# KwonGihyun/TweedieMix

Hardware: AMD Instinct MI355X
Metric: denoise steps/sec @ SDXL 1024^2 K=3 concepts (fusion phase); images/sec at 1/2/4/8 GPUs (higher is better)
Workload: dtype bf16

## Files before the change

### tweediemix_amd/csrc/gemm_kernel.h

```cpp
#pragma once
#include "common.h"
#include <type_traits>
#include <stdlib.h>
#include <atomic>

namespace tmix_gemm {

constexpr int BK = 64;

static __device__ __forceinline__ float xor32_sum(float x) {
    auto r = __builtin_amdgcn_permlane32_swap(__float_as_uint(x), __float_as_uint(x), false, false);
    return __uint_as_float(r[0]) + __uint_as_float(r[1]);
}

template <int CTRL> static __device__ __forceinline__ float dpp_row(float x) {
    return __int_as_float(__builtin_amdgcn_update_dpp(0, __float_as_int(x), CTRL, 0xf, 0xf, false));
}
static __device__ __forceinline__ float swap32_sum(float a, float b) {
    auto r = __builtin_amdgcn_permlane32_swap(__float_as_uint(a), __float_as_uint(b), false, false);
    return __uint_as_float(r[0]) + __uint_as_float(r[1]);
}
static __device__ __forceinline__ float swap16_sum(float a, float b) {
    auto r = __builtin_amdgcn_permlane16_swap(__float_as_uint(a), __float_as_uint(b), false, false);
    return __uint_as_float(r[0]) + __uint_as_float(r[1]);
}

struct Params {
    const bf16_t* A; int64_t lda, strideA;
    const bf16_t* W; int64_t ldw, strideW;
    bf16_t* C; int64_t ldc, strideC;
    const float* bias; int64_t strideBias;
    const bf16_t* R; int64_t ldr, strideR;
    const float* rgb; int rows_per_group;
    bf16_t* Ct; int64_t ldct, strideCt; int n_trans_begin;
    int M, N, K, tiles_m, tiles_n, group_m, epilogue;
    unsigned bytesA, bytesW;
    float* stats_out; int64_t strideStatsOut, ldStatsOut;
    const float* ln_stats; int64_t strideLnStats, ldLnStats; const float* ln_colsum; int64_t strideLnColsum;
    float ln_inv_c, ln_eps; int ln_parts;
    int H, Wd, Cin, Ho, Wo, mode, ntaps;
    int up_hw; unsigned up_magic;
    unsigned long long* prof; int prof_detail;
    int wide;
    const unsigned char* scaleA; const unsigned char* scaleW; int64_t strideScaleA, strideScaleW;
    int64_t ldScaleA;
    unsigned char* scale_out; int64_t ldScaleOut; int f8out;
    unsigned char* f8copy; int64_t ldF8copy;
    const char* pf; long long pf_bytes;
    int pf_per;
    int w_period, w_groups; unsigned w_magic;
    float* cs_out;
    const bf16_t* S1; const bf16_t* S2; int c1s, c2s; unsigned bytesS1, bytesS2;
};

static __device__ __forceinline__ void blds16(__amdgpu_buffer_rsrc_t rsrc, unsigned voff, unsigned soff, char* lds_dst) {
    __builtin_amdgcn_raw_ptr_buffer_load_lds(rsrc, (__attribute__((address_space(3))) void*)lds_dst, 16, voff, soff, 0, 0);
}

constexpr int f8_block_cap(int bn) { return bn >= 256 ? 88 : 224; }

template <int N> static __device__ __forceinline__ void wait_vmcnt() { asm volatile("s_waitcnt vmcnt(%0)" ::"n"(N) : "memory"); }

constexpr int PFU = 8;
#define TMIX_PF_TOUCH(p, pf_keep, touches, nth_, idx)                                                                                                     \
    unsigned pf_keep[PFU];                                                                                                                                \
    _Pragma("unroll") for (int pf_u_ = 0; pf_u_ < PFU; ++pf_u_) pf_keep[pf_u_] = 0;                                                                       \
    if ((p).pf && (touches)) {                                                                                                                            \
        const long long pf_nwg_ = (long long)gridDim.x * gridDim.y, pf_nth_ = (nth_);                                                                     \
        const long long pf_lines_ = ((p).pf_bytes + 127) >> 7; const int pf_per_ = (p).pf_per;                                      \
        const long long pf_first_ = ((long long)blockIdx.y * gridDim.x + blockIdx.x) * pf_nth_ + (idx);                                                   \
        _Pragma("unroll") for (int pf_u_ = 0; pf_u_ < PFU; ++pf_u_) {                                                                                     \
            const long long pf_ln_ = pf_first_ + (long long)pf_u_ * pf_nwg_ * pf_nth_;                                                                    \
            if (pf_u_ < pf_per_ && pf_ln_ < pf_lines_)                                                                                                    \
                asm volatile("global_load_dword %0, %1, off" : "=v"(pf_keep[pf_u_]) : "v"((p).pf + (pf_ln_ << 7)) : "memory");                            \
        }                                                                                                                                                 \
    }
static __device__ __forceinline__ void pf_keep_alive(const unsigned (&pf_keep)[PFU]) {
#pragma unroll
    for (int u = 0; u < PFU; ++u) asm volatile("" :: "v"(pf_keep[u]));
}

struct TileId { int tile_m, tile_n, by; };
static __device__ __forceinline__ TileId tile_of_workgroup(const Params& p) {
    int bid, by;
    xcd_remap_grid(bid, by);
    const int per_group = p.group_m * p.tiles_n;
    const int grp = bid / per_group;
    const int first_m = grp * p.group_m;
    const int gsize = min(p.tiles_m - first_m, p.group_m);
    const int rem = bid - grp * per_group;
    const int tile_n = rem / gsize, tile_m = first_m + (rem - tile_n * gsize);
// ... 334 lines not shown
            }
        }
    };

    if constexpr (LW) {
        if (loader) {
            constexpr int PRE = NS >= 4 ? 2 : NS - 1;
#pragma unroll
            for (int s = 0; s < PRE; ++s)
                if (s < nk) stage(s, s);
            if (nk >= PRE) wait_vmcnt<(PRE - 1) * L>(); else wait_vmcnt<0>();
            pf_keep_alive(pf_keep);
            __builtin_amdgcn_s_barrier();
#pragma unroll
            for (int s = PRE; s < NS - 1; ++s)
                if (s < nk) stage(s, s);
            int nxt = NS - 1;
            for (int kt = 0; kt < nk; ++kt) {
                const bool more = kt + NS - 1 < nk;
                if (more) stage(nxt, kt + NS - 1);
                if (more) wait_vmcnt<(NS - 2) * L>(); else wait_vmcnt<0>();
                __builtin_amdgcn_s_barrier();
                nxt = (nxt + 1 == NS) ? 0 : nxt + 1;
            }
            if (p.stats_out) __syncthreads();
            return;
        }
    }

    uint4* ln_mfrag = (uint4*)(smem + RING);
    uint4* ln_cfrag = ln_mfrag + BM;
    float* ln_rs = (float*)(ln_cfrag + BN);
    float* bias_lds = ln_rs + BM;
    float bias_r = 0.f;
    if (p.bias && tid < BN && n0 + tid < p.N) bias_r = (p.bias + (int64_t)bzw * p.strideBias)[n0 + tid];
    float* rgb_lds = bias_lds + BN;
    float rgb_r = 0.f;
    bool rgb_one = true;
    if constexpr (CONV) {
        if (p.rgb) {
            const int g0 = m0 / p.rows_per_group;
            rgb_one = (min(m0 + BM, p.M) - 1) / p.rows_per_group == g0;
            if (rgb_one && tid < BN && n0 + tid < p.N) rgb_r = p.rgb[(int64_t)g0 * p.N + n0 + tid];
        }
    }
    constexpr int PU = 16;
    typedef __attribute__((ext_vector_type(2))) unsigned u32x2;
    u32x2 lnv[PU];
    float ln_cs = 0.f;
    const bool ln_on = p.ln_stats != nullptr;
    if (ln_on) {
        const __amdgpu_buffer_rsrc_t rsS = __builtin_amdgcn_make_buffer_rsrc((void*)(p.ln_stats + (int64_t)bz * p.strideLnStats), 0,
                                                                              (int)(p.ln_parts * p.ldLnStats * 8), 0x00020000);
        if (tid < BM) {
            const int lnm = min(m0 + tid, p.M - 1);
#pragma unroll
            for (int q = 0; q < PU; ++q)
                if (q < p.ln_parts) lnv[q] = __builtin_amdgcn_raw_buffer_load_b64(rsS, lnm * 8, q * (int)p.ldLnStats * 8, 0);
        }
        if (tid < BN) ln_cs = (p.ln_colsum + (int64_t)bzw * p.strideLnColsum)[min(n0 + tid, p.N - 1)];
    }
    auto ln_reduce = [&]() {
        if (tid < BN) { bias_lds[tid] = bias_r; if constexpr (CONV) rgb_lds[tid] = rgb_r; }
        if (!ln_on) return;
        if (tid < BM) {
            float s1 = 0.f, s2 = 0.f;
#pragma unroll
            for (int q = 0; q < PU; ++q)
                if (q < p.ln_parts) { s1 += __uint_as_float(lnv[q].x); s2 += __uint_as_float(lnv[q].y); }
            const float mean = s1 * p.ln_inv_c;
            ln_rs[tid] = rsqrtf(fmaxf(s2 * p.ln_inv_c - mean * mean, 0.f) + p.ln_eps);
            ln_mfrag[tid] = ln_mean_operand(-mean);
        }
        if (tid < BN) ln_cfrag[tid] = ln_colsum_operand(ln_cs);
    };

    f32x16 acc[FM][FN];
#pragma unroll
    for (int i = 0; i < FM; ++i)
#pragma unroll
        for (int j = 0; j < FN; ++j)
#pragma unroll
            for (int r = 0; r < 16; ++r) acc[i][j][r] = 0.f;

    const bool trans = (EK == 1 || EK == 2 || EK == 4) ? false : (p.n_trans_begin >= 0) && (n0 >= p.n_trans_begin);
    constexpr bool SQ = (FM == FN && TM == TN) && !PH;
    const bool tswap = trans && SQ;
    const int l31 = lane & 31, lhi = lane >> 5;
    const int fsw = (lane >> 1) & 7;

    const int offA = (wr * TM + l31) * 128, offW = A_TILE + (wc * TN + l31) * 128;
    const int off_a = tswap ? offW : offA, off_b = tswap ? offA : offW;
    const bf16_t* Rb = p.R ? p.R + (int64_t)bz * p.strideR : nullptr;
    const bool plain_epi = EK ? false : !trans && p.epilogue != TMIX_EPI_GEGLU && !(p.wide & 1);
    constexpr bool PREF = FM * FN <= 4;
    uint2 rres[PREF ? FM : 1][PREF ? FN : 1][4];
    auto prefetch_residual = [&]() {
        if constexpr (PREF)
#pragma unroll
        for (int i = 0; i < FM; ++i) {
            int m = m0 + wr * TM + i * 32 + l31; if (m > p.M - 1) m = p.M - 1;
#pragma unroll
            for (int j = 0; j < FN; ++j)
#pragma unroll
                for (int g = 0; g < 4; ++g) {
                    int n = n0 + wc * TN + j * 32 + g * 8 + lhi * 4; if (n > p.N - 4) n = p.N - 4;
                    rres[i][j][g] = *(const uint2*)(Rb + (int64_t)m * p.ldr + n);
                }
        }
    };
    constexpr int WP_I = (FN / 2) * 4 + (FN & 1) * 2;
    constexpr bool WPREF = FM * WP_I <= 12 && !(CONV && F8L && LW);
    uint4 rw[WPREF ? FM * WP_I : 1];
    const bool wide_res = EK != 1 && WPREF && Rb && (EK >= 2 || (p.wide & 1)) && kg == 0;
    auto prefetch_residual_wide = [&]() {
        if constexpr (WPREF) {
            auto grab = [&](int j0, int base, auto cf_tag) {
                constexpr int CF = decltype(cf_tag)::value, CW = CF * 32, LPR = CW / 8, RPI = 64 / LPR, NP = 32 / RPI;
                const int rr = lane / LPR, nc = n0 + wc * TN + j0 * 32 + (lane % LPR) * 8;
#pragma unroll
                for (int i = 0; i < FM; ++i)
#pragma unroll
                    for (int ps = 0; ps < NP; ++ps) {
                        const int m = m0 + wr * TM + i * 32 + ps * RPI + rr;
                        if (m < p.M && nc < p.N) rw[i * WP_I + base + ps] = *(const uint4*)(Rb + (int64_t)m * p.ldr + nc);
                    }
            };
#pragma unroll
            for (int c = 0; c < FN / 2; ++c) grab(c * 2, c * 4, std::integral_constant<int, 2>{});
            if constexpr (FN & 1) grab(FN - 1, (FN / 2) * 4, std::integral_constant<int, 1>{});
        }
    };
    auto epi_prefetch = [&]() __attribute__((always_inline)) {
        if constexpr (WPREF) {
            if (wide_res) prefetch_residual_wide();
            else {
#pragma unroll
                for (int q = 0; q < FM * WP_I; ++q) rw[q] = make_uint4(0u, 0u, 0u, 0u);
            }
        }
    };
    if constexpr (PHL) {
        constexpr int PL = PA + PB;
        static_assert(2 * PL <= 63, "vmcnt immediate");
        const int ns = p.K / (64 / EB);
        const int offA4 = (wr * TM + l31) * 64, offW4 = BM * 64 + (wc * TN + l31) * 64;
        typedef int v8i_t __attribute__((ext_vector_type(8)));
        int f8sA[F8 ? FM : 1], f8sW[F8 ? FN : 1];
        if constexpr (F8) {
            const unsigned char* sa = p.scaleA + (int64_t)bz * p.strideScaleA;
            const unsigned char* sw = p.scaleW + (int64_t)bzw * p.strideScaleW;
#pragma unroll
            for (int i = 0; i < FM; ++i) f8sA[i] = F8B ? 0 : (int)(sa[min(m0 + wr * TM + i * 32 + l31, p.M - 1)] * 0x01010101u);
#pragma unroll
            for (int j = 0; j < FN; ++j) f8sW[j] = (int)(sw[min(n0 + wc * TN + j * 32 + l31, p.N - 1)] * 0x01010101u);
        }
        char* const scl = smem + RING + (BM + BN) * 16 + BM * 4 + BN * 4;
        if constexpr (F8B) {
            const int nblk = p.K / 32;
            const __amdgpu_buffer_rsrc_t rsS = __builtin_amdgcn_make_buffer_rsrc((void*)p.scaleA, 0, (int)((int64_t)nblk * p.ldScaleA), 0x00020000);
            const unsigned lane_off = (unsigned)((lane * 16) / BM) * (unsigned)p.ldScaleA + (unsigned)((lane * 16) % BM)
                                    + (unsigned)(bz * p.strideScaleA + m0);
            const int npcs = (nblk * BM + 1023) / 1024;
            for (int q = w; q < npcs; q += NW)
                blds16(rsS, lane_off + (unsigned)(q * (1024 / BM)) * (unsigned)p.ldScaleA, 0u, scl + q * 1024);
        }
        const int f4 = (lane >> 2) & 3;
        const int q0 = ((0 + lhi) ^ f4) << 4, q1 = ((2 + lhi) ^ f4) << 4;
        const int grp = w >> 2;
#pragma unroll
        for (int s = 0; s < 3; ++s)
            if (s < ns) ph_stage(s, s);
        ln_reduce();
        if (ns >= 3) wait_vmcnt<2 * PL>(); else if (ns == 2) wait_vmcnt<PL>(); else wait_vmcnt<0>();
        __builtin_amdgcn_s_barrier();
        asm volatile("" ::: "memory");
        if (prof_on) pt1 = prof_now();
        pf_keep_alive(pf_keep);
        if (grp) { __builtin_amdgcn_s_barrier(); asm volatile("" ::: "memory"); }
        auto slice = [&](int s, auto stage_tag) {
            constexpr bool ST = decltype(stage_tag)::value;
            const char* pa = smem + (s & 3) * SLOT + offA4;
            const char* pw = smem + (s & 3) * SLOT + offW4;
            frag_ab a[2][FM], b[2][FN];
            v8i_t a8[F8 ? FM : 1], b8[F8 ? FN : 1];
            int f8use[F8B ? FM : 1];
            if constexpr (F8) {
                const int c0 = (lhi ^ f4) << 4, c1 = ((2 + lhi) ^ f4) << 4;
#pragma unroll
                for (int i = 0; i < FM; ++i) {
                    const uint4 lo = *(const uint4*)(pa + i * 32 * 64 + c0), hi = *(const uint4*)(pa + i * 32 * 64 + c1);
                    a8[i] = (v8i_t){(int)lo.x, (int)lo.y, (int)lo.z, (int)lo.w, (int)hi.x, (int)hi.y, (int)hi.z, (int)hi.w};
                }
#pragma unroll
                for (int j = 0; j < FN; ++j) {
                    const uint4 lo = *(const uint4*)(pw + j * 32 * 64 + c0), hi = *(const uint4*)(pw + j * 32 * 64 + c1);
                    b8[j] = (v8i_t){(int)lo.x, (int)lo.y, (int)lo.z, (int)lo.w, (int)hi.x, (int)hi.y, (int)hi.z, (int)hi.w};
                }
            } else {
#pragma unroll
            for (int i = 0; i < FM; ++i) { a[0][i] = *(const frag_ab*)(pa + i * 32 * 64 + q0); a[1][i] = *(const frag_ab*)(pa + i * 32 * 64 + q1); }
#pragma unroll
            for (int j = 0; j < FN; ++j) { b[0][j] = *(const frag_ab*)(pw + j * 32 * 64 + q0); b[1][j] = *(const frag_ab*)(pw + j * 32 * 64 + q1); }
            }
            if constexpr (F8B) {
#pragma unroll
                for (int i = 0; i < FM; ++i)
                    f8use[i] = (int)((unsigned)(unsigned char)scl[(2 * s + lhi) * BM + wr * TM + i * 32 + l31] * 0x01010101u);
            }
            if (s + 2 < ns) wait_vmcnt<PL>(); else wait_vmcnt<0>();
            if (PREF && s == ns - 1 && Rb && plain_epi) prefetch_residual();
            if (s == ns - 1) epi_prefetch();
            asm volatile("s_waitcnt lgkmcnt(0)" ::: "memory");
            __builtin_amdgcn_sched_barrier(0);
            __builtin_amdgcn_s_barrier();
            __builtin_amdgcn_sched_barrier(0);
            __builtin_amdgcn_s_setprio(1);
            char* sA = smem + ((s + 3) & 3) * SLOT;
            char* sW = sA + BM * 64;
            constexpr int KSTEPS = F8 ? 1 : 2;
            constexpr int NMF = KSTEPS * FM * FN, GAP = NMF / PL;
            int issued = 0;
#pragma unroll
            for (int kk = 0; kk < KSTEPS; ++kk)
#pragma unroll
                for (int i = 0; i < FM; ++i)
#pragma unroll
                    for (int j = 0; j < FN; ++j) {
                        if constexpr (F8) acc[i][j] = __builtin_amdgcn_mfma_scale_f32_32x32x64_f8f6f4(b8[j], a8[i], acc[i][j], 0, 0, 0, f8sW[j], 0, F8B ? f8use[i] : f8sA[i]);
                        else acc[i][j] = __builtin_amdgcn_mfma_f32_32x32x16_bf16(b[kk][j], a[kk][i], acc[i][j], 0, 0, 0);
                        const int idx = (kk * FM + i) * FN + j;
                        if constexpr (ST) {
                            if (idx % GAP == (GAP > 1 ? 1 : 0) && issued < PL) {
                                __builtin_amdgcn_sched_barrier(0);
                                if (issued < PA) blds16(rsA, phA[issued], (unsigned)(s + 3) * 64u, sA + (issued * NW + w) * 1024);
                                else             blds16(rsW, phW[issued - PA], (unsigned)(s + 3) * 64u, sW + ph_w(issued - PA) * 1024);
                                __builtin_amdgcn_sched_barrier(0);
                                ++issued;
                            }
                        }
                    }
            __builtin_amdgcn_s_setprio(0);
            __builtin_amdgcn_sched_barrier(0);
            __builtin_amdgcn_s_barrier();
            __builtin_amdgcn_sched_barrier(0);
            asm volatile("" ::: "memory");
        };
        int s = 0;
        for (; s + 3 < ns; ++s) slice(s, std::true_type{});
        for (; s < ns; ++s) slice(s, std::false_type{});
        if (!grp) { __builtin_amdgcn_s_barrier(); asm volatile("" ::: "memory"); }
    } else
    {
    if constexpr (!LW) {
#pragma unroll
        for (int s = 0; s < NS - 1; ++s)
            if (s < nk) stage(s, s);
    }
    ln_reduce();
    if constexpr (!LW) { if (nk >= NS - 1) wait_vmcnt<(NS - 2) * L>(); else wait_vmcnt<0>(); }
    __builtin_amdgcn_s_barrier();
    asm volatile("" ::: "memory");
    if (prof_on) pt1 = prof_now();
    pf_keep_alive(pf_keep);
    int cur = 0, nxt = NS - 1;
    constexpr int KPW = F8L ? 2 : 4 / KS;
    const int k0 = kg * KPW;
    typedef int v8i_t __attribute__((ext_vector_type(8)));
    typedef std::conditional_t<F8L, v8i_t, frag_ab> frag_t;
    frag_t fa[2][FM], fb[2][FN];
    int f8a[2][(F8L && F8B) ? FM : 1];
    int f8sA[(F8L && !F8B) ? FM : 1], f8sW[F8L ? FN : 1];
    if constexpr (F8L) {
        const unsigned char* swp_ = p.scaleW + (int64_t)bzw * p.strideScaleW;
#pragma unroll
        for (int j = 0; j < FN; ++j) f8sW[j] = (int)(swp_[min(n0 + wc * TN + j * 32 + l31, p.N - 1)] * 0x01010101u);
        if constexpr (!F8B) {
            const unsigned char* sap_ = p.scaleA + (int64_t)bz * p.strideScaleA;
#pragma unroll
            for (int i = 0; i < FM; ++i) f8sA[i] = (int)(sap_[min(m0 + wr * TM + i * 32 + l31, p.M - 1)] * 0x01010101u);
        }
    }
    auto rdfrag = [&](const char* row, int kk) __attribute__((always_inline)) -> frag_t {
        if constexpr (F8L) {
            const uint4 lo = *(const uint4*)(row + (((4 * kk + lhi) ^ fsw) << 4)), hi = *(const uint4*)(row + (((4 * kk + 2 + lhi) ^ fsw) << 4));
            return (v8i_t){(int)lo.x, (int)lo.y, (int)lo.z, (int)lo.w, (int)hi.x, (int)hi.y, (int)hi.z, (int)hi.w};
        } else {
            return *(const frag_ab*)(row + ((((k0 + kk) * 2 + lhi) ^ fsw) << 4));
        }
    };
    auto rdscale = [&](int rbuf, int kk, int i) __attribute__((always_inline)) -> int {
        if constexpr (CONV) return (int)((unsigned)(unsigned char)smem[rbuf * STAGE + A_TILE + B_TILE + (wr * TM + i * 32 + l31) * 4 + 2 * kk + lhi] * 0x01010101u);
        else return (int)((unsigned)(unsigned char)smem[rbuf * STAGE + A_TILE + B_TILE + (2 * kk + lhi) * BM + wr * TM + i * 32 + l31] * 0x01010101u);
    };
    auto mma = [&](f32x16& c, const frag_t& b_, const frag_t& a_, int j, int i, int S) __attribute__((always_inline)) {
        if constexpr (F8L) c = __builtin_amdgcn_mfma_scale_f32_32x32x64_f8f6f4(b_, a_, c, 0, 0, 0, f8sW[j], 0, F8B ? f8a[S][F8B ? i : 0] : f8sA[F8B ? 0 : i]);
        else c = __builtin_amdgcn_mfma_f32_32x32x16_bf16(b_, a_, c, 0, 0, 0);
    };
    constexpr int NMF = FM * FN, NRD = FM + FN;
    constexpr bool ROLL = (NW * KS > 4 && NMF * 16 + 2 * NRD * 4 > 200) || (F8L && LW);
    auto kstep = [&](const int S, const int rbuf, const int rkk, const int nd, const int dbuf, const int dkt) {
        const char* pa = smem + rbuf * STAGE + off_a;
        const char* pb = smem + rbuf * STAGE + off_b;
        char* sA = smem + dbuf * STAGE;
        constexpr int RPQ = (NRD + NMF - 1) / NMF;
        const int dpq = (nd + NMF - 1) / NMF;
#pragma unroll
        for (int q = 0; q < NMF; ++q) {
            const int i = ROLL ? q % FM : q / FN, j = ROLL ? q / FM : q - (q / FN) * FN;
            const int SB = ROLL ? 0 : S;
            mma(acc[i][j], fb[SB][j], fa[S][i], j, i, S);
            __builtin_amdgcn_sched_barrier(0);
            if constexpr (ROLL) {
                if (q < FM) { fa[1 - S][q] = rdfrag(pa + q * 32 * 128, rkk); if constexpr (F8L && F8B) f8a[1 - S][q] = rdscale(rbuf, rkk, q); }
                if (i == FM - 1) fb[0][j] = rdfrag(pb + j * 32 * 128, rkk);
            } else {
#pragma unroll
                for (int u = 0; u < RPQ; ++u) {
                    const int r = q * RPQ + u;
                    if (r < FM) { fa[1 - S][r] = rdfrag(pa + r * 32 * 128, rkk); if constexpr (F8L && F8B) f8a[1 - S][r] = rdscale(rbuf, rkk, r); }
                    else if (r < NRD) fb[1 - S][r - FM] = rdfrag(pb + (r - FM) * 32 * 128, rkk);
                }
            }
            if constexpr (!CONV && !LW) {
#pragma unroll
                for (int u = 0; u < dpq; ++u) {
                    const int r = q * dpq + u;
                    if (r < nd) dma_piece(r, sA, dkt);
                }
            }
            __builtin_amdgcn_sched_barrier(0);
        }
    };
    auto ktile = [&](int kt, auto more_tag) {
        constexpr bool MORE = decltype(more_tag)::value && !LW;
        if constexpr (CONV && MORE) { stage(nxt, kt + NS - 1); __builtin_amdgcn_sched_barrier(0); }
        if constexpr (!decltype(more_tag)::value) {
            if (PREF && kt == nk - 1 && Rb && plain_epi) prefetch_residual();
            if (kt == nk - 1) epi_prefetch();
            __builtin_amdgcn_sched_barrier(0);
        }
#pragma unroll
        for (int kk = 0; kk < KPW - 1; ++kk)
            kstep(kk & 1, cur, kk + 1, (kk == 0 && MORE && !CONV) ? L : 0, nxt, kt + NS - 1);
        if constexpr (KPW == 1 && !CONV && MORE) { stage(nxt, kt + NS - 1); __builtin_amdgcn_sched_barrier(0); }
        asm volatile("s_waitcnt lgkmcnt(0)" ::: "memory");
        if constexpr (!LW) { if constexpr (MORE) wait_vmcnt<(NS - 2) * L>(); else { if (kt + 1 < nk) wait_vmcnt<0>(); } }
        __builtin_amdgcn_sched_barrier(0);
        __builtin_amdgcn_s_barrier();
        __builtin_amdgcn_sched_barrier(0);
        asm volatile("" ::: "memory");
        cur = (cur + 1 == NS) ? 0 : cur + 1;
        nxt = (nxt + 1 == NS) ? 0 : nxt + 1;
        kstep((KPW - 1) & 1, cur, 0, 0, 0, 0);
    };
    static_assert(KPW == 1 || ((KPW - 1) & 1) == 1, "the next tile's first fragments go to register set 0");
#pragma unroll
    for (int r = 0; r < NRD; ++r) {
        if (r < FM) { fa[0][r] = rdfrag(smem + off_a + r * 32 * 128, 0); if constexpr (F8L && F8B) f8a[0][r] = rdscale(0, 0, r); }
        else fb[0][r - FM] = rdfrag(smem + off_b + (r - FM) * 32 * 128, 0);
    }
    int kt = 0;
    for (; kt + NS - 1 < nk; ++kt) ktile(kt, std::true_type{});
    for (; kt < nk; ++kt) ktile(kt, std::false_type{});
    }

    if constexpr (KS > 1) {
        float4* xch = (float4*)smem + (size_t)wm_ * (FM * FN * 4 * 64) + lane;
        if (kg == 1) {
#pragma unroll
            for (int i = 0; i < FM; ++i)
#pragma unroll
                for (int j = 0; j < FN; ++j)
#pragma unroll
                    for (int g = 0; g < 4; ++g)
                        xch[((i * FN + j) * 4 + g) * 64] = make_float4(acc[i][j][g * 4], acc[i][j][g * 4 + 1], acc[i][j][g * 4 + 2], acc[i][j][g * 4 + 3]);
        }
        __syncthreads();
        if (kg == 1) {
            __syncthreads();
            if (p.stats_out) __syncthreads();
            return;
        }
#pragma unroll
        for (int i = 0; i < FM; ++i)
#pragma unroll
            for (int j = 0; j < FN; ++j)
#pragma unroll
                for (int g = 0; g < 4; ++g) {
                    const float4 v = xch[((i * FN + j) * 4 + g) * 64];
                    acc[i][j][g * 4] += v.x; acc[i][j][g * 4 + 1] += v.y; acc[i][j][g * 4 + 2] += v.z; acc[i][j][g * 4 + 3] += v.w;
                }
        __syncthreads();
    }
    if (prof_on) pt2 = prof_now();
    float rs_row[FM];
#pragma unroll
    for (int i = 0; i < FM; ++i) rs_row[i] = 1.f;
    if (p.ln_stats) {
        const uint2* srcA = (const uint2*)(ln_mfrag + wr * TM + l31) + lhi;
        const uint2* srcW = (const uint2*)(ln_cfrag + wc * TN + l31) + lhi;
        const uint2* src_a = tswap ? srcW : srcA;
        const uint2* src_b = tswap ? srcA : srcW;
        frag_ab fa[FM], fb[FN];
#pragma unroll
        for (int i = 0; i < FM; ++i) {
            const uint2 h = src_a[i * 64];
            uint4 u = make_uint4(h.x, h.y, 0u, 0u);
            fa[i] = *(frag_ab*)&u;
            if (!tswap) rs_row[i] = ln_rs[wr * TM + i * 32 + l31];
        }
#pragma unroll
        for (int j = 0; j < FN; ++j) {
            const uint2 h = src_b[j * 64];
            uint4 u = make_uint4(h.x, h.y, 0u, 0u);
            fb[j] = *(frag_ab*)&u;
        }
#pragma unroll
        for (int i = 0; i < FM; ++i)
#pragma unroll
            for (int j = 0; j < FN; ++j)
                acc[i][j] = __builtin_amdgcn_mfma_f32_32x32x16_bf16(fb[j], fa[i], acc[i][j], 0, 0, 0);
    }

    const float* bias = p.bias ? p.bias + (int64_t)bzw * p.strideBias : nullptr;
    constexpr int STG_MAX = 32 * (2 * 32 * 4 + 16);
    if (trans) {
        if constexpr (!SQ) {
            bf16_t* Ct = p.Ct + (int64_t)bz * p.strideCt;
            constexpr int SR = FM * 64 + 16, LPR = FM * 4, RPI = 64 / LPR, NP = 32 / RPI;
            static_assert(32 * SR <= STG_MAX && 64 % LPR == 0, "transposed staging patch");
            char* stg = smem + w * STG_MAX;
            const int rr = lane / LPR, cc = (lane % LPR) * 8;
#pragma unroll
            for (int j = 0; j < FN; ++j) {
                const int nb = n0 + wc * TN + j * 32;
#pragma unroll
                for (int g = 0; g < 4; ++g) {
                    float bv[4] = {0.f, 0.f, 0.f, 0.f};
                    if (bias && nb < p.N) { const float4 b4 = *(const float4*)(bias + nb + g * 8 + lhi * 4); bv[0] = b4.x; bv[1] = b4.y; bv[2] = b4.z; bv[3] = b4.w; }
#pragma unroll
                    for (int i = 0; i < FM; ++i)
#pragma unroll
                        for (int r = 0; r < 4; ++r)
                            *(bf16_t*)(stg + (g * 8 + lhi * 4 + r) * SR + (i * 32 + l31) * 2) = f2bf(fmaf(acc[i][j][g * 4 + r], rs_row[i], bv[r]));
                }
#pragma unroll
                for (int ps = 0; ps < NP; ++ps) {
                    const int r = ps * RPI + rr, n = nb + r, m = m0 + wr * TM + cc;
                    const uint4 v = *(const uint4*)(stg + r * SR + cc * 2);
                    if (n >= p.N || m >= p.M) continue;
                    bf16_t* dst = Ct + (int64_t)(n - p.n_trans_begin) * p.ldct + m;
                    if (m + 8 <= p.M) *(uint4*)dst = v;
                    else {
                        const unsigned u[4] = {v.x, v.y, v.z, v.w};
                        for (int k = 0; k < 8 && m + k < p.M; ++k) dst[k] = (bf16_t)(u[k >> 1] >> ((k & 1) * 16));
                    }
                }
            }
            if (prof_on) prof_leave(p.prof, p.prof_detail, pt0, pt1, pt2);
            return;
        }
        if constexpr (SQ) {
            bf16_t* Ct = p.Ct + (int64_t)bz * p.strideCt;
            if (EK == 3 || (p.wide & 4)) {
                constexpr int CF = (FN % 2 == 0) ? 2 : 1, SR = CF * 64 + 16, LPR = CF * 4, RPI = 64 / LPR, NP = 32 / RPI;
                char* stg = smem + w * STG_MAX;
                const int rr = lane / LPR, cc = (lane % LPR) * 8;
#pragma unroll
                for (int i = 0; i < FM; ++i) {
                    const int nl = n0 + wc * TN + i * 32 + l31;
                    const float bv = (bias && nl < p.N) ? bias[nl] : 0.f;
#pragma unroll
                    for (int c = 0; c < FN / CF; ++c) {
#pragma unroll
                        for (int jj = 0; jj < CF; ++jj)
#pragma unroll
                            for (int g = 0; g < 4; ++g) {
                                const int j = c * CF + jj, ml = wr * TM + j * 32 + g * 8 + lhi * 4;
                                const float4 rs = p.ln_stats ? *(const float4*)(ln_rs + ml) : make_float4(1.f, 1.f, 1.f, 1.f);
                                uint2 v;
                                v.x = pack_bf2(fmaf(acc[i][j][g * 4 + 0], rs.x, bv), fmaf(acc[i][j][g * 4 + 1], rs.y, bv));
                                v.y = pack_bf2(fmaf(acc[i][j][g * 4 + 2], rs.z, bv), fmaf(acc[i][j][g * 4 + 3], rs.w, bv));
                                *(uint2*)(stg + l31 * SR + (jj * 32 + g * 8 + lhi * 4) * 2) = v;
                            }
#pragma unroll
                        for (int ps = 0; ps < NP; ++ps) {
                            const int r = ps * RPI + rr, n = n0 + wc * TN + i * 32 + r, m = m0 + wr * TM + c * CF * 32 + cc;
                            const uint4 v = *(const uint4*)(stg + r * SR + cc * 2);
                            if (n >= p.N || m >= p.M) continue;
                            bf16_t* dst = Ct + (int64_t)(n - p.n_trans_begin) * p.ldct + m;
                            if (m + 8 <= p.M) *(uint4*)dst = v;
                            else {
                                const unsigned u[4] = {v.x, v.y, v.z, v.w};
                                for (int k = 0; k < 8 && m + k < p.M; ++k) dst[k] = (bf16_t)(u[k >> 1] >> ((k & 1) * 16));
                            }
                        }
                    }
                }
                if (prof_on) prof_leave(p.prof, p.prof_detail, pt0, pt1, pt2);
                return;
            }
#pragma unroll
            for (int i = 0; i < FM; ++i) {
                const int n = n0 + wc * TN + i * 32 + l31;
                if (n >= p.N) continue;
                const float bv = bias ? bias[n] : 0.f;
                bf16_t* row = Ct + (int64_t)(n - p.n_trans_begin) * p.ldct;
#pragma unroll
                for (int j = 0; j < FN; ++j)
#pragma unroll
                    for (int g = 0; g < 4; ++g) {
                        const int ml = wr * TM + j * 32 + g * 8 + lhi * 4, m = m0 + ml;
                        if (m >= p.M) continue;
                        const float4 rs = p.ln_stats ? *(const float4*)(ln_rs + ml) : make_float4(1.f, 1.f, 1.f, 1.f);
                        const float o0 = fmaf(acc[i][j][g * 4 + 0], rs.x, bv), o1 = fmaf(acc[i][j][g * 4 + 1], rs.y, bv);
                        const float o2 = fmaf(acc[i][j][g * 4 + 2], rs.z, bv), o3 = fmaf(acc[i][j][g * 4 + 3], rs.w, bv);
                        if (m + 3 < p.M && ((p.ldct & 3) == 0)) {
                            uint2 v;
                            v.x = pack_bf2(o0, o1);
                            v.y = pack_bf2(o2, o3);
                            *(uint2*)(row + m) = v;
                        } else {
                            const float o[4] = {o0, o1, o2, o3};
#pragma unroll
                            for (int r = 0; r < 4; ++r) if (m + r < p.M) row[m + r] = f2bf(o[r]);
                        }
                    }
            }
        }
        if (prof_on) prof_leave(p.prof, p.prof_detail, pt0, pt1, pt2);
        return;
    }

    bf16_t* Cb = p.C + (int64_t)bz * p.strideC;
    int up_mb = 0, up_ob = 0;
    if constexpr (CONV) {
        if (upf) { up_mb = up_q * p.up_hw; up_ob = ((up_q >> 2) * p.Ho + ((up_q >> 1) & 1)) * p.Wo + (up_q & 1); }
    }
    auto conv_store_row = [&](int m) __attribute__((always_inline)) -> int {
        if constexpr (CONV) {
            if (upf) {
                const unsigned l = (unsigned)(m - up_mb), sy = __umulhi(l, p.up_magic), sx = l - sy * (unsigned)p.Wd;
                return up_ob + (int)(2u * sy * (unsigned)p.Wo + 2u * sx);
            }
        }
        return m;
    };
    if (EK == 1 || (EK == 0 && p.epilogue == TMIX_EPI_GEGLU)) {
        if (EK == 1 || (p.wide & 2)) {
            char* stg = smem + w * STG_MAX;
            auto chunk = [&](int i, int j0, auto cf_tag) {
                constexpr int CF = decltype(cf_tag)::value, OC = CF * 16, SR = OC * 2 + 16, LPR = OC / 8, RPI = 64 / LPR, NP = 32 / RPI;
                const int rr = lane / LPR, cc = (lane % LPR) * 8;
#pragma unroll
                for (int jj = 0; jj < CF; ++jj) {
                    const int j = j0 + jj;
#pragma unroll
                    for (int g = 0; g < 2; ++g) {
                        float o[4];
                        const float4 ba = *(const float4*)(bias_lds + wc * TN + j * 32 + g * 8 + lhi * 4), bg = *(const float4*)(bias_lds + wc * TN + j * 32 + g * 8 + lhi * 4 + 16);
                        const float bav[4] = {ba.x, ba.y, ba.z, ba.w}, bgv[4] = {bg.x, bg.y, bg.z, bg.w};
#pragma unroll
                        for (int r = 0; r < 4; ++r) {
                            const float a = fmaf(acc[i][j][g * 4 + r], rs_row[i], bav[r]), gt = fmaf(acc[i][j][(g + 2) * 4 + r], rs_row[i], bgv[r]);
                            o[r] = a * gelu_erf_f(gt);
                        }
                        uint2 v; v.x = pack_bf2(o[0], o[1]); v.y = pack_bf2(o[2], o[3]);
                        *(uint2*)(stg + l31 * SR + (jj * 16 + g * 8 + lhi * 4) * 2) = v;
                    }
                }
#pragma unroll
                for (int ps = 0; ps < NP; ++ps) {
                    const int r = ps * RPI + rr, m = m0 + wr * TM + i * 32 + r;
                    const uint4 v = *(const uint4*)(stg + r * SR + cc * 2);
                    const int nb = n0 + wc * TN + (j0 + cc / 16) * 32;
                    const int col = (n0 + wc * TN) / 2 + j0 * 16 + cc;
                    if constexpr (CF >= 2) {
                        if (p.f8out) {
                            const unsigned u[4] = {v.x, v.y, v.z, v.w};
                            float f[8], am = 0.f;
#pragma unroll
                            for (int k = 0; k < 4; ++k) { f[2 * k] = __uint_as_float(u[k] << 16); f[2 * k + 1] = __uint_as_float(u[k] & 0xffff0000u);
                                                          am = fmaxf(am, fmaxf(fabsf(f[2 * k]), fabsf(f[2 * k + 1]))); }
                            const MxPacked mx = mx_pack8(f, quad_max(am));
                            if (m >= p.M || nb >= p.N) continue;
                            *(uint2*)((unsigned char*)p.C + (int64_t)bz * p.strideC + (int64_t)m * p.ldc + col) = make_uint2(mx.lo, mx.hi);
                            if ((lane & 3) == 0) p.scale_out[(int64_t)(col >> 5) * p.ldScaleOut + (int64_t)bz * p.M + m] = (unsigned char)(mx.e + 127);
                            continue;
                        }
                    }
                    if (m >= p.M || nb >= p.N) continue;
                    *(uint4*)(Cb + (int64_t)m * p.ldc + col) = v;
                }
            };
#pragma unroll
            for (int i = 0; i < FM; ++i) {
                constexpr int C4 = FN / 4, R4 = FN % 4;
#pragma unroll
                for (int c = 0; c < C4; ++c) chunk(i, c * 4, std::integral_constant<int, 4>{});
                if constexpr (R4 >= 2) chunk(i, C4 * 4, std::integral_constant<int, 2>{});
                if constexpr (R4 & 1) chunk(i, FN - 1, std::integral_constant<int, 1>{});
            }
            if (prof_on) prof_leave(p.prof, p.prof_detail, pt0, pt1, pt2);
            return;
        }
#pragma unroll
        for (int i = 0; i < FM; ++i) {
            const int m = m0 + wr * TM + i * 32 + l31;
            if (m >= p.M) continue;
#pragma unroll
            for (int j = 0; j < FN; ++j) {
                const int nb = n0 + wc * TN + j * 32;
                if (nb >= p.N) continue;
#pragma unroll
                for (int g = 0; g < 2; ++g) {
                    const int nv = nb + g * 8 + lhi * 4;
                    float o[4];
#pragma unroll
                    for (int r = 0; r < 4; ++r) {
                        float a = acc[i][j][g * 4 + r], gt = acc[i][j][(g + 2) * 4 + r];
                        if (bias) { a = fmaf(a, rs_row[i], bias[nv + r]); gt = fmaf(gt, rs_row[i], bias[nv + 16 + r]); }
                        else { a *= rs_row[i]; gt *= rs_row[i]; }
                        o[r] = a * gelu_erf_f(gt);
                    }
                    uint2 v; v.x = pack_bf2(o[0], o[1]); v.y = pack_bf2(o[2], o[3]);
                    *(uint2*)(Cb + (int64_t)m * p.ldc + nb / 2 + g * 8 + lhi * 4) = v;
                }
            }
        }
        if (prof_on) prof_leave(p.prof, p.prof_detail, pt0, pt1, pt2);
        return;
    }
    float2* sto = (!CONV && p.stats_out) ? (float2*)(p.stats_out + (int64_t)bz * p.strideStatsOut) : nullptr;
    if (EK >= 2 || (p.wide & 1)) {
        char* stg = smem + w * STG_MAX;
        float2* redw = (float2*)(smem + NW * STG_MAX);
        const bool f32out = p.epilogue == TMIX_EPI_F32OUT;
        float sa1[FM][4], sa2[FM][4], sb1[FM][2], sb2[FM][2];
#pragma unroll
        for (int i = 0; i < FM; ++i) {
#pragma unroll
            for (int q = 0; q < 4; ++q) { sa1[i][q] = 0.f; sa2[i][q] = 0.f; }
            sb1[i][0] = sb1[i][1] = sb2[i][0] = sb2[i][1] = 0.f;
        }
        auto cs_flush = [&](float (&cv)[16], int mb, int nc, bool ncok, auto cf_tag) __attribute__((always_inline)) {
            constexpr int CF = decltype(cf_tag)::value;
            float t[8], u[4];
#pragma unroll
            for (int k = 0; k < 8; ++k) t[k] = swap32_sum(cv[k], cv[8 + k]);
#pragma unroll
            for (int k = 0; k < 4; ++k) u[k] = swap16_sum(t[k], t[k + 4]);
#pragma unroll
            for (int k = 0; k < 4; ++k) u[k] += dpp_row<0x128>(u[k]);
            if constexpr (CF == 1) {
#pragma unroll
                for (int k = 0; k < 4; ++k) u[k] += dpp_row<0x124>(u[k]);
            }
            if (!(lane & (CF == 1 ? 12 : 8)) && mb < p.M && ncok)
                *(float4*)(p.cs_out + ((int64_t)(mb >> 5) * 2 + (lane >> 5)) * p.N + nc + ((lane >> 4) & 1) * 4) = make_float4(u[0], u[1], u[2], u[3]);
        };
        auto cs_add = [&](float (&cv)[16], const uint4& v) __attribute__((always_inline)) {
            const unsigned u[4] = {v.x, v.y, v.z, v.w};
#pragma unroll
            for (int k = 0; k < 4; ++k) {
                const float lo = __uint_as_float(u[k] << 16), hi = __uint_as_float(u[k] & 0xffff0000u);
                cv[2 * k] += lo; cv[2 * k + 1] += hi;
                cv[8 + 2 * k] = fmaf(lo, lo, cv[8 + 2 * k]); cv[9 + 2 * k] = fmaf(hi, hi, cv[9 + 2 * k]);
            }
        };
        auto chunk = [&](int j0, auto cf_tag, auto fl_tag) __attribute__((always_inline)) {
            constexpr int CF = decltype(cf_tag)::value, CW = CF * 32, SR = CW * 4 + 16, LPR = CW / 8, RPI = 64 / LPR, NP = 32 / RPI;
            constexpr int FL = decltype(fl_tag)::value;
            const int rr = lane / LPR, cc = (lane % LPR) * 8;
            const int nc = n0 + wc * TN + j0 * 32 + cc;
            const bool ncok = nc < p.N;
            if constexpr ((FL & 1) != 0) {
                constexpr int CI = CF == 2 ? 0 : (FN / 2) * 4;
                const bool lnf = p.ln_stats != nullptr;
                const float4 bq0 = *(const float4*)(bias_lds + wc * TN + j0 * 32 + cc), bq1 = *(const float4*)(bias_lds + wc * TN + j0 * 32 + cc + 4);
                const float bq[8] = {bq0.x, bq0.y, bq0.z, bq0.w, bq1.x, bq1.y, bq1.z, bq1.w};
                float tq[8];
                if constexpr (CONV) {
                    const float4 t0 = *(const float4*)(rgb_lds + wc * TN + j0 * 32 + cc), t1 = *(const float4*)(rgb_lds + wc * TN + j0 * 32 + cc + 4);
                    tq[0] = t0.x; tq[1] = t0.y; tq[2] = t0.z; tq[3] = t0.w; tq[4] = t1.x; tq[5] = t1.y; tq[6] = t1.z; tq[7] = t1.w;
                }
#pragma unroll
                for (int i = 0; i < FM; ++i) {
                    const int mb = m0 + wr * TM + i * 32;
                    float cv[(FL & 8) ? 16 : 1];
                    if constexpr ((FL & 8) != 0) {
#pragma unroll
                        for (int k = 0; k < 16; ++k) cv[k] = 0.f;
                    }
#pragma unroll
                    for (int jj = 0; jj < CF; ++jj)
#pragma unroll
                        for (int g = 0; g < 4; ++g)
                            *(float4*)(stg + l31 * SR + (jj * 32 + g * 8 + lhi * 4) * 4) =
                                make_float4(acc[i][j0 + jj][g * 4 + 0], acc[i][j0 + jj][g * 4 + 1], acc[i][j0 + jj][g * 4 + 2], acc[i][j0 + jj][g * 4 + 3]);
#pragma unroll
                    for (int ps = 0; ps < NP; ++ps) {
                        const int r = ps * RPI + rr, m = mb + r;
                        const float4 v0 = *(const float4*)(stg + r * SR + cc * 4), v1 = *(const float4*)(stg + r * SR + cc * 4 + 16);
                        const float rsl = ln_rs[wr * TM + i * 32 + r];
                        const float rs = lnf ? rsl : 1.f;
                        float o[8] = {v0.x, v0.y, v0.z, v0.w, v1.x, v1.y, v1.z, v1.w};
#pragma unroll
                        for (int k = 0; k < 8; ++k) o[k] = fmaf(o[k], rs, bq[k]);
                        if constexpr (CONV) {
#pragma unroll
                            for (int k = 0; k < 8; ++k) o[k] += tq[k];
                        }
                        if constexpr (WPREF) {
                            const uint4 rq = rw[i * WP_I + CI + (CF == 2 ? (j0 / 2) * 4 : 0) + ps];
                            const unsigned ru[4] = {rq.x, rq.y, rq.z, rq.w};
#pragma unroll
                            for (int k = 0; k < 4; ++k) { o[2 * k] += __uint_as_float(ru[k] << 16); o[2 * k + 1] += __uint_as_float(ru[k] & 0xffff0000u); }
                        }
                        uint4 v;
                        v.x = pack_bf2(o[0], o[1]); v.y = pack_bf2(o[2], o[3]); v.z = pack_bf2(o[4], o[5]); v.w = pack_bf2(o[6], o[7]);
                        const bool ok = m < p.M && ncok;
                        if (ok) *(uint4*)(Cb + (int64_t)conv_store_row(m) * p.ldc + nc) = v;
                        if constexpr (F8C && (FL & 4) != 0) {
                            const unsigned u8[4] = {v.x, v.y, v.z, v.w};
                            float f[8], am = 0.f;
#pragma unroll
                            for (int k = 0; k < 4; ++k) { f[2 * k] = __uint_as_float(u8[k] << 16); f[2 * k + 1] = __uint_as_float(u8[k] & 0xffff0000u);
                                                          am = fmaxf(am, fmaxf(fabsf(f[2 * k]), fabsf(f[2 * k + 1]))); }
                            const MxPacked mx = mx_pack8(f, quad_max(am));
                            if (ok) {
                                *(uint2*)(p.f8copy + ((int64_t)bz * p.M + m) * p.ldF8copy + nc) = make_uint2(mx.lo, mx.hi);
                                if ((lane & 3) == 0) p.scale_out[(int64_t)(nc >> 5) * p.ldScaleOut + (int64_t)bz * p.M + m] = (unsigned char)(mx.e + 127);
                            }
                        }
                        if constexpr ((FL & 2) != 0) {
                            const unsigned u[4] = {v.x, v.y, v.z, v.w};
                            float a1 = 0.f, a2 = 0.f;
#pragma unroll
                            for (int k = 0; k < 4; ++k) {
                                const float lo = __uint_as_float(u[k] << 16), hi = __uint_as_float(u[k] & 0xffff0000u);
                                a1 += lo + hi; a2 = fmaf(lo, lo, a2); a2 = fmaf(hi, hi, a2);
                            }
                            if (!ok) { a1 = 0.f; a2 = 0.f; }
                            if constexpr (CF == 2) { sa1[i][ps] += a1; sa2[i][ps] += a2; } else { sb1[i][ps] += a1; sb2[i][ps] += a2; }
                        }
                        if constexpr ((FL & 8) != 0) cs_add(cv, v);
                    }
                    if constexpr ((FL & 8) != 0) cs_flush(cv, mb, nc, ncok, cf_tag);
                }
                return;
            }
            float bv[8];
#pragma unroll
            for (int k = 0; k < 8; ++k) bv[k] = 0.f;
            if (bias && ncok) {
                const float4 b0 = *(const float4*)(bias + nc), b1 = *(const float4*)(bias + nc + 4);
                bv[0] = b0.x; bv[1] = b0.y; bv[2] = b0.z; bv[3] = b0.w; bv[4] = b1.x; bv[5] = b1.y; bv[6] = b1.z; bv[7] = b1.w;
            }
#pragma unroll
            for (int i = 0; i < FM; ++i) {
                const int mb = m0 + wr * TM + i * 32;
                float cv[(FL & 8) ? 16 : 1];
                if constexpr ((FL & 8) != 0) {
#pragma unroll
                    for (int k = 0; k < 16; ++k) cv[k] = 0.f;
                }
                uint4 rv[NP];
                if (Rb) {
#pragma unroll
                    for (int ps = 0; ps < NP; ++ps) {
                        const int m = mb + ps * RPI + rr;
                        if constexpr (WPREF) rv[ps] = rw[i * WP_I + (CF == 2 ? (j0 / 2) * 4 : (FN / 2) * 4) + ps];
                        else if (m < p.M && ncok) rv[ps] = *(const uint4*)(Rb + (int64_t)m * p.ldr + nc);
                    }
                }
#pragma unroll
                for (int jj = 0; jj < CF; ++jj)
#pragma unroll
                    for (int g = 0; g < 4; ++g)
                        *(float4*)(stg + l31 * SR + (jj * 32 + g * 8 + lhi * 4) * 4) =
                            make_float4(acc[i][j0 + jj][g * 4 + 0], acc[i][j0 + jj][g * 4 + 1], acc[i][j0 + jj][g * 4 + 2], acc[i][j0 + jj][g * 4 + 3]);
#pragma unroll
                for (int ps = 0; ps < NP; ++ps) {
                    const int r = ps * RPI + rr, m = mb + r;
                    const float4 v0 = *(const float4*)(stg + r * SR + cc * 4), v1 = *(const float4*)(stg + r * SR + cc * 4 + 16);
                    if (m >= p.M || !ncok) continue;
                    float o[8] = {v0.x, v0.y, v0.z, v0.w, v1.x, v1.y, v1.z, v1.w};
                    if (bias) { const float rs = p.ln_stats ? ln_rs[wr * TM + i * 32 + r] : 1.f;
#pragma unroll
                                for (int k = 0; k < 8; ++k) o[k] = fmaf(o[k], rs, bv[k]); }
                    else if (p.ln_stats) { const float rs = ln_rs[wr * TM + i * 32 + r];
#pragma unroll
                                for (int k = 0; k < 8; ++k) o[k] *= rs; }
                    if (p.rgb) {
                        const float* rg = p.rgb + (int64_t)(m / p.rows_per_group) * p.N + nc;
                        const float4 b0 = *(const float4*)rg, b1 = *(const float4*)(rg + 4);
                        o[0] += b0.x; o[1] += b0.y; o[2] += b0.z; o[3] += b0.w; o[4] += b1.x; o[5] += b1.y; o[6] += b1.z; o[7] += b1.w;
                    }
                    if (p.epilogue == TMIX_EPI_GELU) {
#pragma unroll
                        for (int k = 0; k < 8; ++k) o[k] = gelu_erf_f(o[k]);
                    } else if (p.epilogue == TMIX_EPI_QUICKGELU) {
#pragma unroll
                        for (int k = 0; k < 8; ++k) o[k] = o[k] * __builtin_amdgcn_rcpf(1.0f + __builtin_amdgcn_exp2f(-2.4554669595930157f * o[k]));
                    }
                    if (Rb) {
                        const unsigned u[4] = {rv[ps].x, rv[ps].y, rv[ps].z, rv[ps].w};
#pragma unroll
                        for (int k = 0; k < 4; ++k) { o[2 * k] += bf2f((bf16_t)(u[k] & 0xffff)); o[2 * k + 1] += bf2f((bf16_t)(u[k] >> 16)); }
                    }
                    if (f32out) {
                        float* dst = (float*)p.C + (int64_t)bz * p.strideC + (int64_t)m * p.ldc + nc;
                        *(float4*)dst = make_float4(o[0], o[1], o[2], o[3]);
                        *(float4*)(dst + 4) = make_float4(o[4], o[5], o[6], o[7]);
                    } else {
                        uint4 v;
                        v.x = pack_bf2(o[0], o[1]); v.y = pack_bf2(o[2], o[3]); v.z = pack_bf2(o[4], o[5]); v.w = pack_bf2(o[6], o[7]);
                        *(uint4*)(Cb + (int64_t)conv_store_row(m) * p.ldc + nc) = v;
                        if constexpr (F8C) if (p.f8copy) {
                            const unsigned u8[4] = {v.x, v.y, v.z, v.w};
                            float f[8], am = 0.f;
#pragma unroll
                            for (int k = 0; k < 4; ++k) { f[2 * k] = __uint_as_float(u8[k] << 16); f[2 * k + 1] = __uint_as_float(u8[k] & 0xffff0000u);
                                                          am = fmaxf(am, fmaxf(fabsf(f[2 * k]), fabsf(f[2 * k + 1]))); }
                            const MxPacked mx = mx_pack8(f, quad_max(am));
                            *(uint2*)(p.f8copy + ((int64_t)bz * p.M + m) * p.ldF8copy + nc) = make_uint2(mx.lo, mx.hi);
                            if ((lane & 3) == 0) p.scale_out[(int64_t)(nc >> 5) * p.ldScaleOut + (int64_t)bz * p.M + m] = (unsigned char)(mx.e + 127);
                        }
                        if (sto) {
                            const unsigned u[4] = {v.x, v.y, v.z, v.w};
                            float a1 = 0.f, a2 = 0.f;
#pragma unroll
                            for (int k = 0; k < 4; ++k) {
                                const float lo = __uint_as_float(u[k] << 16), hi = __uint_as_float(u[k] & 0xffff0000u);
                                a1 += lo + hi; a2 = fmaf(lo, lo, a2); a2 = fmaf(hi, hi, a2);
                            }
                            if constexpr (CF == 2) { sa1[i][ps] += a1; sa2[i][ps] += a2; } else { sb1[i][ps] += a1; sb2[i][ps] += a2; }
                        }
                        if constexpr ((FL & 8) != 0) cs_add(cv, v);
                    }
                }
                if constexpr ((FL & 8) != 0) cs_flush(cv, mb, nc, ncok, cf_tag);
            }
        };
        constexpr int C2 = FN / 2;
        auto chunks = [&](auto fl_tag) __attribute__((always_inline)) {
#pragma unroll
            for (int c = 0; c < C2; ++c) chunk(c * 2, std::integral_constant<int, 2>{}, fl_tag);
            if constexpr (FN & 1) chunk(FN - 1, std::integral_constant<int, 1>{}, fl_tag);
        };
        const bool fastp = (WPREF || !Rb) && !f32out && p.epilogue == TMIX_EPI_NONE && (!p.rgb || (CONV && rgb_one));
        bool f8q = false;
        if constexpr (F8C) f8q = p.f8copy != nullptr;
        if constexpr (EK == 4) { if constexpr (F8C) { if (!sto) chunks(std::integral_constant<int, 5>{}); else chunks(std::integral_constant<int, 7>{}); } }
        else if constexpr (CS) { if (!fastp) chunks(std::integral_constant<int, 8>{}); else chunks(std::integral_constant<int, 9>{}); }
        else if (!fastp) chunks(std::integral_constant<int, 0>{});
        else if (!f8q) { if (!sto) chunks(std::integral_constant<int, 1>{}); else chunks(std::integral_constant<int, 3>{}); }
        else { if constexpr (F8C) { if (!sto) chunks(std::integral_constant<int, 5>{}); else chunks(std::integral_constant<int, 7>{}); } }
// ... 145 lines not shown
```

Measured before the change: 32.94.

## Use 16x16x32 bf16 MFMA path for phased 256x320 GEGLU/LN GEMM tiles

Adds an alternate compute path for phased 256x320 tiles with EK 1 or 2: the main loop issues 16x16x32 bf16 MFMAs with their own LDS fragment addressing, and B fragments are loaded a few steps ahead. The LayerNorm mean correction and the GEGLU and plain epilogues are rewritten to read the new f32x4 accumulator layout. The path is on by default through a macro. The aim is a better MFMA/LDS schedule or lower register pressure for this tile shape. The cost is a second accumulator array and more instructions per K-slice, since 16x16 MFMAs do less work per instruction.

New measurement: 33.01 (median of 4 runs). About the same (+0.2%).

```diff
diff --git a/tweediemix_amd/csrc/gemm_kernel.h b/tweediemix_amd/csrc/gemm_kernel.h
--- a/tweediemix_amd/csrc/gemm_kernel.h
+++ b/tweediemix_amd/csrc/gemm_kernel.h
@@ -7,6 +7,9 @@
 namespace tmix_gemm {
 
 constexpr int BK = 64;
+#ifndef TMIX_PH320_MFMA16
+#define TMIX_PH320_MFMA16 1
+#endif
 
 static __device__ __forceinline__ float xor32_sum(float x) {
     auto r = __builtin_amdgcn_permlane32_swap(__float_as_uint(x), __float_as_uint(x), false, false);
@@ -507,6 +510,14 @@
         for (int j = 0; j < FN; ++j)
 #pragma unroll
             for (int r = 0; r < 16; ++r) acc[i][j][r] = 0.f;
+    constexpr bool M16 = PH == 1 && BM == 256 && BN == 320 && (EK == 1 || EK == 2) && TMIX_PH320_MFMA16;
+    constexpr int FM4 = M16 ? TM / 16 : 1, FN4 = M16 ? TN / 16 : 1;
+    f32x4 acc4[FM4][FN4];
+#pragma unroll
+    for (int i = 0; i < FM4; ++i)
+#pragma unroll
+        for (int j = 0; j < FN4; ++j) acc4[i][j] = (f32x4){0.f, 0.f, 0.f, 0.f};
+    const int l15 = lane & 15, lg = lane >> 4;
 
     const bool trans = (EK == 1 || EK == 2 || EK == 4) ? false : (p.n_trans_begin >= 0) && (n0 >= p.n_trans_begin);
     constexpr bool SQ = (FM == FN && TM == TN) && !PH;
@@ -592,6 +603,7 @@
         }
         const int f4 = (lane >> 2) & 3;
         const int q0 = ((0 + lhi) ^ f4) << 4, q1 = ((2 + lhi) ^ f4) << 4;
+        const int kch = ((lg & 1) * 3) ^ (lg >> 1);
         const int grp = w >> 2;
 #pragma unroll
         for (int s = 0; s < 3; ++s)
@@ -608,6 +620,10 @@
             const char* pa = smem + (s & 3) * SLOT + offA4;
             const char* pw = smem + (s & 3) * SLOT + offW4;
             frag_ab a[2][FM], b[2][FN];
+            frag_ab a16[FM4], b16[FN4];
+            constexpr int WAH = 2;
+            const char* pa16 = smem + (s & 3) * SLOT + (wr * TM + l15) * 64 + ((kch ^ f4) << 4);
+            const char* pw16 = smem + (s & 3) * SLOT + BM * 64 + (wc * TN + l15) * 64 + ((kch ^ f4) << 4);
             v8i_t a8[F8 ? FM : 1], b8[F8 ? FN : 1];
             int f8use[F8B ? FM : 1];
             if constexpr (F8) {
@@ -622,6 +638,11 @@
                     const uint4 lo = *(const uint4*)(pw + j * 32 * 64 + c0), hi = *(const uint4*)(pw + j * 32 * 64 + c1);
                     b8[j] = (v8i_t){(int)lo.x, (int)lo.y, (int)lo.z, (int)lo.w, (int)hi.x, (int)hi.y, (int)hi.z, (int)hi.w};
                 }
+            } else if constexpr (M16) {
+#pragma unroll
+                for (int i = 0; i < FM4; ++i) a16[i] = *(const frag_ab*)(pa16 + i * 16 * 64);
+#pragma unroll
+                for (int j = 0; j < WAH; ++j) b16[j] = *(const frag_ab*)(pw16 + j * 16 * 64);
             } else {
 #pragma unroll
             for (int i = 0; i < FM; ++i) { a[0][i] = *(const frag_ab*)(pa + i * 32 * 64 + q0); a[1][i] = *(const frag_ab*)(pa + i * 32 * 64 + q1); }
@@ -646,6 +667,30 @@
             constexpr int KSTEPS = F8 ? 1 : 2;
             constexpr int NMF = KSTEPS * FM * FN, GAP = NMF / PL;
             int issued = 0;
+            if constexpr (M16) {
+                constexpr int NMF16 = FM4 * FN4, GAP16 = NMF16 / PL;
+#pragma unroll
+                for (int j = 0; j < FN4; ++j)
+#pragma unroll
+                    for (int i = 0; i < FM4; ++i) {
+                        acc4[i][j] = __builtin_amdgcn_mfma_f32_16x16x32_bf16(b16[j], a16[i], acc4[i][j], 0, 0, 0);
+                        const int idx = j * FM4 + i;
+                        if (i == 0 && j + WAH < FN4) {
+                            __builtin_amdgcn_sched_barrier(0);
+                            b16[j + WAH] = *(const frag_ab*)(pw16 + (j + WAH) * 16 * 64);
+                            __builtin_amdgcn_sched_barrier(0);
+                        }
+                        if constexpr (ST) {
+                            if (idx % GAP16 == 1 && issued < PL) {
+                                __builtin_amdgcn_sched_barrier(0);
+                                if (issued < PA) blds16(rsA, phA[issued], (unsigned)(s + 3) * 64u, sA + (issued * NW + w) * 1024);
+                                else             blds16(rsW, phW[issued - PA], (unsigned)(s + 3) * 64u, sW + ph_w(issued - PA) * 1024);
+                                __builtin_amdgcn_sched_barrier(0);
+                                ++issued;
+                            }
+                        }
+                    }
+            } else {
 #pragma unroll
             for (int kk = 0; kk < KSTEPS; ++kk)
 #pragma unroll
@@ -665,6 +710,7 @@
                             }
                         }
                     }
+            }
             __builtin_amdgcn_s_setprio(0);
             __builtin_amdgcn_sched_barrier(0);
             __builtin_amdgcn_s_barrier();
@@ -822,6 +868,37 @@
     float rs_row[FM];
 #pragma unroll
     for (int i = 0; i < FM; ++i) rs_row[i] = 1.f;
+    float rs16[FM4];
+#pragma unroll
+    for (int i = 0; i < FM4; ++i) rs16[i] = (M16 && p.ln_stats) ? ln_rs[wr * TM + i * 16 + l15] : 1.f;
+    if constexpr (M16) {
+        if (p.ln_stats) {
+            frag_ab la[FM4], lb[FN4];
+#pragma unroll
+            for (int i = 0; i < FM4; ++i) {
+                uint2 h = make_uint2(0u, 0u);
+                if (lg < 2) h = ((const uint2*)(ln_mfrag + wr * TM + i * 16 + l15))[lg];
+                uint4 u = make_uint4(h.x, h.y, 0u, 0u);
+                la[i] = *(frag_ab*)&u;
+            }
+            auto ln_col = [&](int j) __attribute__((always_inline)) {
+                uint2 h = make_uint2(0u, 0u);
+                if (lg < 2) h = ((const uint2*)(ln_cfrag + wc * TN + j * 16 + l15))[lg];
+                uint4 u = make_uint4(h.x, h.y, 0u, 0u);
+                lb[j] = *(frag_ab*)&u;
+            };
+            ln_col(0);
+#pragma unroll
+            for (int j = 0; j < FN4; ++j) {
+                if (j + 1 < FN4) ln_col(j + 1);
+                __builtin_amdgcn_sched_barrier(0);
+#pragma unroll
+                for (int i = 0; i < FM4; ++i)
+                    acc4[i][j] = __builtin_amdgcn_mfma_f32_16x16x32_bf16(lb[j], la[i], acc4[i][j], 0, 0, 0);
+                __builtin_amdgcn_sched_barrier(0);
+            }
+        }
+    } else
     if (p.ln_stats) {
         const uint2* srcA = (const uint2*)(ln_mfrag + wr * TM + l31) + lhi;
         const uint2* srcW = (const uint2*)(ln_cfrag + wc * TN + l31) + lhi;
@@ -978,6 +1055,25 @@
             auto chunk = [&](int i, int j0, auto cf_tag) {
                 constexpr int CF = decltype(cf_tag)::value, OC = CF * 16, SR = OC * 2 + 16, LPR = OC / 8, RPI = 64 / LPR, NP = 32 / RPI;
                 const int rr = lane / LPR, cc = (lane % LPR) * 8;
+                if constexpr (M16) {
+#pragma unroll
+                    for (int jj = 0; jj < CF; ++jj) {
+                        const int j = j0 + jj;
+                        const float4 ba = *(const float4*)(bias_lds + wc * TN + j * 32 + lg * 4), bg = *(const float4*)(bias_lds + wc * TN + j * 32 + lg * 4 + 16);
+                        const float bav[4] = {ba.x, ba.y, ba.z, ba.w}, bgv[4] = {bg.x, bg.y, bg.z, bg.w};
+#pragma unroll
+                        for (int h = 0; h < 2; ++h) {
+                            float o[4];
+#pragma unroll
+                            for (int r = 0; r < 4; ++r) {
+                                const float a = fmaf(acc4[2 * i + h][2 * j][r], rs16[2 * i + h], bav[r]), gt = fmaf(acc4[2 * i + h][2 * j + 1][r], rs16[2 * i + h], bgv[r]);
+                                o[r] = a * gelu_erf_f(gt);
+                            }
+                            uint2 v; v.x = pack_bf2(o[0], o[1]); v.y = pack_bf2(o[2], o[3]);
+                            *(uint2*)(stg + (h * 16 + l15) * SR + (jj * 16 + lg * 4) * 2) = v;
+                        }
+                    }
+                } else
 #pragma unroll
                 for (int jj = 0; jj < CF; ++jj) {
                     const int j = j0 + jj;
@@ -1118,6 +1214,13 @@
 #pragma unroll
                         for (int k = 0; k < 16; ++k) cv[k] = 0.f;
                     }
+                    if constexpr (M16) {
+#pragma unroll
+                        for (int h = 0; h < 2; ++h)
+#pragma unroll
+                            for (int q = 0; q < 2 * CF; ++q)
+                                *(f32x4*)(stg + (h * 16 + l15) * SR + (q * 16 + lg * 4) * 4) = acc4[2 * i + h][2 * j0 + q];
+                    } else
 #pragma unroll
                     for (int jj = 0; jj < CF; ++jj)
 #pragma unroll
@@ -1171,6 +1274,7 @@
                             if constexpr (CF == 2) { sa1[i][ps] += a1; sa2[i][ps] += a2; } else { sb1[i][ps] += a1; sb2[i][ps] += a2; }
                         }
                         if constexpr ((FL & 8) != 0) cs_add(cv, v);
+                        if constexpr (M16) __builtin_amdgcn_sched_barrier(0);
                     }
                     if constexpr ((FL & 8) != 0) cs_flush(cv, mb, nc, ncok, cf_tag);
                 }
@@ -1200,6 +1304,13 @@
                         else if (m < p.M && ncok) rv[ps] = *(const uint4*)(Rb + (int64_t)m * p.ldr + nc);
                     }
                 }
+                if constexpr (M16) {
+#pragma unroll
+                    for (int h = 0; h < 2; ++h)
+#pragma unroll
+                        for (int q = 0; q < 2 * CF; ++q)
+                            *(f32x4*)(stg + (h * 16 + l15) * SR + (q * 16 + lg * 4) * 4) = acc4[2 * i + h][2 * j0 + q];
+                } else
 #pragma unroll
                 for (int jj = 0; jj < CF; ++jj)
 #pragma unroll
```
